# peleiden/librubiks

Hardware: AMD Instinct MI355X
Metric: cube node-expansions/sec (12-child fan-out) at 1M-state batch (higher is better)
Workload: dtype u8

## Files before the change

librubiks_amd/csrc/rk_mcts.hip:

```cpp
#include <hip/hip_runtime.h>
#include <algorithm>
#include <climits>
#include <cmath>
#include <cstdlib>
#include <cstring>
#include <vector>

#include "../../include/rubiks_hip.h"
#include "rk_device.h"
#include "rk_error.h"
#include "rk_kernels.h"

namespace rk {

struct MctsDev {
	int T;
	uint32_t cap1;
	uint32_t tmask;
	uint32_t max_path;
	double c, nu;
	uint32_t *states;
	uint8_t *nodes;
	uint32_t *table;
	int32_t *path_nodes; uint8_t *path_actions;
	int32_t *tree;
	uint32_t *children; int32_t *child_idx; uint8_t *child_new;
};

enum { TR_PLEN = 0, TR_NSTATES, TR_MAXSTATES, TR_SIMS, TR_SOLVE_ACTION, TR_SOLVE_LEAF, TR_READY, TR_FLAGS , TR_INTS = 8 };
enum { MCTS_ERR_PATH = 1, MCTS_ERR_LINK = 2, MCTS_ERR_NOT_EXPANDED = 3 };
__host__ __device__ inline int flags_done(int f) { return f & 0xFF; }
__host__ __device__ inline int flags_solved(int f) { return (f >> 8) & 0xFF; }
__host__ __device__ inline int flags_error(int f) { return (f >> 16) & 0xFF; }

struct TreeRec { int32_t v[TR_INTS]; };

__device__ __forceinline__ TreeRec load_tree(const int32_t *tree, int t)
{
	const u32x4 a = reinterpret_cast<const u32x4 *>(tree)[2 * t], b = reinterpret_cast<const u32x4 *>(tree)[2 * t + 1];
	return TreeRec{{(int32_t)a.x, (int32_t)a.y, (int32_t)a.z, (int32_t)a.w, (int32_t)b.x, (int32_t)b.y, (int32_t)b.z, (int32_t)b.w}};
}

constexpr int NODE_BYTES = 512;
constexpr int OFF_EXPANDED = 0, OFF_V = 8, OFF_N = 16, OFF_NB = 64, OFF_P = 112, OFF_W = 208, OFF_L = 304, OFF_STAMP = 400, OFF_SUMN = 448, OFF_SQRTN = 456;

struct Node {
	uint8_t *p;
	__device__ __forceinline__ uint32_t &expanded() const { return *reinterpret_cast<uint32_t *>(p + OFF_EXPANDED); }
	__device__ __forceinline__ double &V() const { return *reinterpret_cast<double *>(p + OFF_V); }
	__device__ __forceinline__ int32_t *N() const { return reinterpret_cast<int32_t *>(p + OFF_N); }
	__device__ __forceinline__ int32_t *nb() const { return reinterpret_cast<int32_t *>(p + OFF_NB); }
	__device__ __forceinline__ double *P() const { return reinterpret_cast<double *>(p + OFF_P); }
	__device__ __forceinline__ double *W() const { return reinterpret_cast<double *>(p + OFF_W); }
	__device__ __forceinline__ double *L() const { return reinterpret_cast<double *>(p + OFF_L); }
	__device__ __forceinline__ int32_t *stamp() const { return reinterpret_cast<int32_t *>(p + OFF_STAMP); }
	__device__ __forceinline__ int32_t *sumN() const { return reinterpret_cast<int32_t *>(p + OFF_SUMN); }
	__device__ __forceinline__ double &sqrtN() const { return *reinterpret_cast<double *>(p + OFF_SQRTN); }
};

__device__ __forceinline__ Node node_of(const MctsDev &d, size_t node0, int idx)
{
	return Node{d.nodes + (node0 + (size_t)idx) * NODE_BYTES};
}

__device__ __forceinline__ uint32_t mcts_hash(const uint32_t s[5])
{
	uint64_t h = 0x9E3779B97F4A7C15ull;
	#pragma unroll
	for (int j = 0; j < 5; j++) {
		h ^= s[j];
		h *= 0xFF51AFD7ED558CCDull;
		h ^= h >> 29;
	}
	return (uint32_t)(h ^ (h >> 32));
}

__device__ __forceinline__ bool same5(const uint32_t a[5], const uint32_t *p)
{
	return ((a[0] ^ p[0]) | (a[1] ^ p[1]) | (a[2] ^ p[2]) | (a[3] ^ p[3]) | (a[4] ^ p[4])) == 0;
}

template <int N> __device__ __forceinline__ int dpp_ror_i(int v)
{
	return __builtin_amdgcn_update_dpp(v, v, 0x120 + N, 0xF, 0xF, false);
}
template <int N> __device__ __forceinline__ double dpp_ror_d(double v)
{
	const long long b = __double_as_longlong(v);
	const int lo = dpp_ror_i<N>((int)(b & 0xFFFFFFFFll)), hi = dpp_ror_i<N>((int)(b >> 32));
	return __longlong_as_double(((long long)hi << 32) | (unsigned int)lo);
}
__device__ __forceinline__ int row_sum_i(int v)
{
	v += dpp_ror_i<8>(v); v += dpp_ror_i<4>(v); v += dpp_ror_i<2>(v); v += dpp_ror_i<1>(v);
	return v;
}
__device__ __forceinline__ float row_max_f(float v)
{
	#define RK_STEP(N) v = fmaxf(v, __int_as_float(dpp_ror_i<N>(__float_as_int(v))))
	RK_STEP(8); RK_STEP(4); RK_STEP(2); RK_STEP(1);
	#undef RK_STEP
	return v;
}
template <int N> __device__ __forceinline__ double dpp_ror_d_fresh(double v)
{
	const long long b = __double_as_longlong(v);
	const int lo = __builtin_amdgcn_mov_dpp((int)(b & 0xFFFFFFFFll), 0x120 + N, 0xF, 0xF, false);
	const int hi = __builtin_amdgcn_mov_dpp((int)(b >> 32), 0x120 + N, 0xF, 0xF, false);
	return __longlong_as_double(((long long)hi << 32) | (unsigned int)lo);
}
__device__ __forceinline__ double max_f64_raw(double a, double b)
{
	double r;
	asm("v_max_f64 %0, %1, %2" : "=v"(r) : "v"(a), "v"(b));
	return r;
}
__device__ __forceinline__ double row_max_d(double v)
{
	#define RK_STEP(N) v = max_f64_raw(v, dpp_ror_d_fresh<N>(v))
	RK_STEP(8); RK_STEP(4); RK_STEP(2); RK_STEP(1);
	#undef RK_STEP
	return v;
}
__device__ __forceinline__ void fence_wave_to_wave()
{
	__builtin_amdgcn_fence(__ATOMIC_RELEASE, "workgroup");
	__builtin_amdgcn_fence(__ATOMIC_ACQUIRE, "workgroup");
}

__global__ __launch_bounds__(64)
void k_mcts_root(MctsDev d, const uint32_t *starts, const int32_t *max_states)
{
	const int t = blockIdx.x, lane = threadIdx.x;
	uint32_t s[5];
	#pragma unroll
	for (int j = 0; j < 5; j++) s[j] = starts[(size_t)t * 5 + j];
	if (lane == 0) {
		uint32_t *st = d.states + ((size_t)t * d.cap1 + 1) * 5;
		#pragma unroll
		for (int j = 0; j < 5; j++) st[j] = s[j];
		d.table[(size_t)t * (d.tmask + 1) + (mcts_hash(s) & d.tmask)] = 1u;
		int32_t *tr = d.tree + (size_t)t * TR_INTS;
		tr[TR_NSTATES] = 1;
		tr[TR_MAXSTATES] = max_states[t];
		d.path_nodes[(size_t)t * d.max_path] = 1;
		tr[TR_PLEN] = 1;
		tr[TR_SIMS] = 0;
		tr[TR_READY] = 0;
		tr[TR_SOLVE_ACTION] = -1;
		tr[TR_SOLVE_LEAF] = -1;
		const bool solved = is_solved5(s);
		tr[TR_FLAGS] = solved ? (1 | (2 << 8)) : 0;
	}
}

__global__ void k_mcts_set_root_pv(MctsDev d, const float *probs, const float *values)
{
	const int i = blockIdx.x * blockDim.x + threadIdx.x;
	if (i >= d.T * 12) return;
	const int t = i / 12, k = i - 12 * t;
	const Node root = node_of(d, (size_t)t * d.cap1, 1);
	root.P()[k] = (double)probs[i];
	if (k == 0) root.V() = (double)values[t];
}

__global__ void k_mcts_gather_roots(MctsDev d, uint32_t *out)
{
	const int i = blockIdx.x * blockDim.x + threadIdx.x;
	if (i >= d.T * 5) return;
	const int t = i / 5, j = i - 5 * t;
	out[i] = d.states[((size_t)t * d.cap1 + 1) * 5 + j];
}

__device__ __forceinline__ void expand_leaf_body(const MctsDev &d, const u32x4 *s_act, int t, int lane, int n, int max_states, int flags, int leaf)
{
	const bool active = lane < 12;
	const size_t cbase = (size_t)t * 12 + lane;
	int32_t *trw = d.tree + (size_t)t * TR_INTS;
	if (n + 12 > max_states) {
		if (active) d.child_new[cbase] = 0;
		if (lane == 0) { trw[TR_FLAGS] = flags | 1; trw[TR_READY] = 1; }
		return;
	}
	const size_t node0 = (size_t)t * d.cap1;
	uint32_t s[5];
	#pragma unroll
	for (int j = 0; j < 5; j++) s[j] = d.states[(node0 + leaf) * 5 + j];
	uint32_t tab[12];
	load_action_table(s_act, active ? (uint32_t)lane : 0u, tab);
	move5(s, tab);

	uint32_t *table = d.table + (size_t)t * (d.tmask + 1);
	uint32_t slot = mcts_hash(s) & d.tmask;
	int idx = 0;
	if (active) {
		for (;;) {
			const uint32_t e = table[slot];
			if (e == 0u) break;
			if (same5(s, d.states + (node0 + e) * 5)) { idx = (int)e; break; }
			slot = (slot + 1) & d.tmask;
		}
	}
	const bool is_new = active && idx == 0;
	const unsigned long long newmask = __ballot(is_new);
	if (is_new) {
		idx = n + 1 + __popcll(newmask & ((1ull << lane) - 1ull));
		while (atomicCAS(&table[slot], 0u, (uint32_t)idx) != 0u) slot = (slot + 1) & d.tmask;
		#pragma unroll
		for (int j = 0; j < 5; j++) d.states[(node0 + idx) * 5 + j] = s[j];
	}
	if (active) {
		#pragma unroll
		for (int j = 0; j < 5; j++) d.children[cbase * 5 + j] = s[j];
		d.child_idx[cbase] = idx;
		d.child_new[cbase] = is_new ? 1 : 0;
		node_of(d, node0, leaf).nb()[lane] = idx;
		node_of(d, node0, idx).nb()[lane ^ 1] = leaf;
	}
	const unsigned long long solvedmask = __ballot(active && is_solved5(s));
	if (solvedmask != 0ull && lane == __ffsll((long long)solvedmask) - 1) {
		trw[TR_FLAGS] = (flags & 0xFF) | (1 << 8);
		trw[TR_SOLVE_ACTION] = lane;
		trw[TR_SOLVE_LEAF] = idx;
	}
	if (lane == 0) {
		node_of(d, node0, leaf).expanded() = 1u;
		trw[TR_NSTATES] = n + __popcll(newmask);
		trw[TR_READY] = 1;
	}
}

__global__ __launch_bounds__(64)
void k_mcts_expand(MctsDev d)
{
	__shared__ u32x4 s_act[36];
	const int t = blockIdx.x, lane = threadIdx.x;
	stage_action_tables(s_act, lane);
	__syncthreads();
	const TreeRec tr = load_tree(d.tree, t);
	if (tr.v[TR_FLAGS] & 0xFF) {
		if (lane < 12) d.child_new[(size_t)t * 12 + lane] = 0;
		return;
	}
	if (tr.v[TR_READY]) return;
	const int leaf = d.path_nodes[(size_t)t * d.max_path + tr.v[TR_PLEN] - 1];
	expand_leaf_body(d, s_act, t, lane, tr.v[TR_NSTATES], tr.v[TR_MAXSTATES], tr.v[TR_FLAGS], leaf);
}

template <int IN>
__device__ __forceinline__ float net_scalar(const void *p, size_t i)
{
	if (IN == 2) return __builtin_bit_cast(float, (uint32_t)reinterpret_cast<const uint16_t *>(p)[i] << 16);
	return reinterpret_cast<const float *>(p)[i];
}

template <int IN>
__device__ __forceinline__ void child_policy(const void *probs, size_t row, int stride, float out[12])
{
	#pragma unroll
	for (int k = 0; k < 12; k++) out[k] = net_scalar<IN>(probs, row * (size_t)stride + k);
	if (IN == 0) return;
	float m = out[0];
	#pragma unroll
	for (int k = 1; k < 12; k++) m = out[k] > m ? out[k] : m;
	#pragma unroll
	for (int k = 0; k < 12; k++) out[k] = expf(out[k] - m);
	const float a0 = (out[0] + out[8]) + out[4], a1 = (out[1] + out[9]) + out[5];
	const float a2 = (out[2] + out[10]) + out[6], a3 = (out[3] + out[11]) + out[7];
	const float sum = (a0 + a2) + (a1 + a3);
	#pragma unroll
	for (int k = 0; k < 12; k++) out[k] = out[k] / sum;
}

template <int IN>
__global__ __launch_bounds__(64)
void k_mcts_backup_select(MctsDev d, const void *probs, const void *values, int p_stride, int v_stride, int ahead_limit, int first_tree)
{
	__shared__ u32x4 s_act[36];
	const int t = blockIdx.x + first_tree, lane = threadIdx.x;
	if (ahead_limit != 0) stage_action_tables(s_act, lane);
	const bool active = lane < 12;
	const size_t node0 = (size_t)t * d.cap1;
	const size_t cbase = (size_t)t * 12 + lane;
	const int32_t *pnodes = d.path_nodes + (size_t)t * d.max_path;
	uint8_t *pacts = d.path_actions + (size_t)t * d.max_path;
	const TreeRec tr = load_tree(d.tree, t);
	int32_t *trw = d.tree + (size_t)t * TR_INTS;
	const int is_done = flags_done(tr.v[TR_FLAGS]), tree_solved = flags_solved(tr.v[TR_FLAGS]);
	const int plen = tr.v[TR_PLEN], sims_before = tr.v[TR_SIMS];
	const int idx = active ? d.child_idx[cbase] : 0;
	const bool is_new = active && d.child_new[cbase] != 0;
	const size_t rbase = (size_t)blockIdx.x * 12 + lane;
	const float vf = active ? net_scalar<IN>(values, rbase * (size_t)v_stride) : 0.0f;
	if (is_done) {
		if (ahead_limit != 0 && active) d.child_new[cbase] = 0;
		return;
	}
	if (!tr.v[TR_READY]) {
		if (lane == 0) trw[TR_FLAGS] = tr.v[TR_FLAGS] | 1 | (MCTS_ERR_NOT_EXPANDED << 16);
		return;
	}
	if (lane == 0) trw[TR_READY] = 0;
	const int leaf = pnodes[plen - 1];
	const double v = (double)vf;
	if (is_new) {
		const Node child = node_of(d, node0, idx);
		child.V() = v;
		float pk[12];
		child_policy<IN>(probs, rbase, p_stride, pk);
		#pragma unroll
		for (int k = 0; k < 12; k++) {
			child.P()[k] = (double)pk[k];
			child.W()[k] = v;
		}
	}
	float bestf = is_new ? vf : -INFINITY;
	bestf = __int_as_float(__builtin_amdgcn_readfirstlane(__float_as_int(row_max_f(bestf))));
	const bool has_new = __ballot(is_new) != 0ull;
	const double best = (double)bestf;
	if (active) node_of(d, node0, leaf).W()[lane] = is_new ? v : node_of(d, node0, idx).V();

	const int sim = sims_before + 1;
	for (int e = lane; e < plen - 1; e += 64) {
		const int act = pacts[e];
		const Node nd = node_of(d, node0, pnodes[e]);
		const double w = nd.W()[act];
		const int cnt = nd.N()[act];
		const int last = atomicExch(&nd.stamp()[act], sim);
		if (has_new && best > w) nd.W()[act] = best;
		if (last != sim) {
			nd.N()[act] = cnt + 1;
			const int total = atomicAdd(nd.sumN(), 1) + 1;
			atomicMax(reinterpret_cast<unsigned long long *>(&nd.sqrtN()), (unsigned long long)__double_as_longlong(sqrt((double)total)));
		}
		nd.L()[act] = 0.0;
		node_of(d, node0, pnodes[e + 1]).L()[act ^ 1] = 0.0;
	}
	if (lane == 0) trw[TR_SIMS] = sim;
	if (tree_solved) {
		if (lane == 0) {
			pacts[plen - 1] = (uint8_t)tr.v[TR_SOLVE_ACTION];
			trw[TR_FLAGS] = tr.v[TR_FLAGS] | 1;
		}
		if (ahead_limit != 0 && active) d.child_new[cbase] = 0;
		return;
	}
	fence_wave_to_wave();

	int cur = 1, len = 1, owed_lane = -1;
	for (;;) {
		const Node nd = node_of(d, node0, cur);
		const int col = lane < 12 ? lane : 11;
		const uint32_t expanded = nd.expanded();
		const double sqrtN = nd.sqrtN();
		const int nA = nd.N()[col];
		const double pA = nd.P()[col], wA = nd.W()[col];
		double lval = nd.L()[col];
		const int nb = nd.nb()[col];
		if (lane == owed_lane) { lval += d.nu; nd.L()[col] = lval; }
		if (!expanded) break;
		double x = -INFINITY;
		int best_a;
		{
			double U = d.c * pA;
			U = U * sqrtN;
			U = U / (double)(1 + nA);
			const double Q = wA - lval;
			x = active ? U + Q : -INFINITY;
		}
		const double mx = row_max_d(x);
		best_a = __ffsll((long long)(__ballot(x == mx) & 0xFFFull)) - 1;
		const int next = __builtin_amdgcn_readlane(nb, best_a);
		if (lane == best_a) nd.L()[col] = lval + d.nu;
		owed_lane = best_a ^ 1;
		if (lane == 0) {
			pacts[len - 1] = (uint8_t)best_a;
			d.path_nodes[(size_t)t * d.max_path + len] = next;
		}
		len++;
		cur = next;
		if (len >= (int)d.max_path || next <= 0) {
			if (lane == 0) trw[TR_FLAGS] = tr.v[TR_FLAGS] | 1 | ((next <= 0 ? MCTS_ERR_LINK : MCTS_ERR_PATH) << 16);
			break;
		}
	}
	if (lane == 0) trw[TR_PLEN] = len;
	const bool broke_on_error = len >= (int)d.max_path || cur <= 0;
	if (ahead_limit != 0 && !broke_on_error && (ahead_limit < 0 || sim < ahead_limit)) {
		fence_wave_to_wave();
		expand_leaf_body(d, s_act, t, lane, tr.v[TR_NSTATES], tr.v[TR_MAXSTATES], tr.v[TR_FLAGS], cur);
	} else if (ahead_limit != 0 && active) {
		d.child_new[cbase] = 0;
	}
}


__global__ __launch_bounds__(256)
void k_mcts_rehash(MctsDev d)
{
	const int t = blockIdx.y;
	const int n = d.tree[(size_t)t * TR_INTS + TR_NSTATES];
	const size_t node0 = (size_t)t * d.cap1;
	uint32_t *table = d.table + (size_t)t * (d.tmask + 1);
	for (int idx = 1 + blockIdx.x * blockDim.x + threadIdx.x; idx <= n; idx += gridDim.x * blockDim.x) {
		uint32_t s[5];
		#pragma unroll
		for (int j = 0; j < 5; j++) s[j] = d.states[(node0 + idx) * 5 + j];
		uint32_t slot = mcts_hash(s) & d.tmask;
		while (atomicCAS(&table[slot], 0u, (uint32_t)idx) != 0u) slot = (slot + 1) & d.tmask;
	}
}

__global__ void k_mcts_set_budgets(MctsDev d, const int32_t *max_states)
{
	const int t = blockIdx.x * blockDim.x + threadIdx.x;
	if (t >= d.T) return;
	int32_t *tr = d.tree + (size_t)t * TR_INTS;
	tr[TR_MAXSTATES] = max_states[t];
	const int f = tr[TR_FLAGS];
	if (flags_done(f) && !flags_solved(f) && !flags_error(f) && tr[TR_NSTATES] + 12 <= max_states[t]) {
		tr[TR_FLAGS] = f & ~0xFF;
		tr[TR_READY] = 0;
	}
}

__global__ __launch_bounds__(256)
void k_mcts_complete(MctsDev d)
{
	__shared__ u32x4 s_act[36];
	stage_action_tables(s_act, threadIdx.x);
	__syncthreads();
	const int t = blockIdx.y;
	const int32_t *tr = d.tree + (size_t)t * TR_INTS;
	if (flags_solved(tr[TR_FLAGS]) != 1) return;
	const int n = tr[TR_NSTATES];
	const size_t node0 = (size_t)t * d.cap1;
	const uint32_t *table = d.table + (size_t)t * (d.tmask + 1);
	const int a = threadIdx.x & 15;
	for (int idx = 1 + (blockIdx.x * blockDim.x + threadIdx.x) / 16; idx <= n; idx += gridDim.x * blockDim.x / 16) {
		const Node leaf = node_of(d, node0, idx);
		if (a >= 12 || leaf.expanded()) continue;
		uint32_t s[5];
		#pragma unroll
		for (int j = 0; j < 5; j++) s[j] = d.states[(node0 + idx) * 5 + j];
		uint32_t tab[12];
		load_action_table(s_act, (uint32_t)a, tab);
		move5(s, tab);
		uint32_t slot = mcts_hash(s) & d.tmask;
		int child = 0;
		for (;;) {
			const uint32_t e = table[slot];
			if (e == 0u) break;
			if (same5(s, d.states + (node0 + e) * 5)) { child = (int)e; break; }
			slot = (slot + 1) & d.tmask;
		}
		leaf.nb()[a] = child;
		if (child) node_of(d, node0, child).nb()[a ^ 1] = idx;
	}
}

struct BfsDev {
	uint32_t *claim;
	int32_t *from;
	uint8_t *act;
	int32_t *front[2];
	int32_t *len;
	uint8_t *actions;
};

__device__ __forceinline__ int ld_i32(const int32_t *p) { return __hip_atomic_load(p, __ATOMIC_RELAXED, __HIP_MEMORY_SCOPE_AGENT); }
__device__ __forceinline__ uint32_t ld_u32(const uint32_t *p) { return __hip_atomic_load(p, __ATOMIC_RELAXED, __HIP_MEMORY_SCOPE_AGENT); }

__global__ __launch_bounds__(1024)
void k_mcts_bfs(MctsDev d, BfsDev b)
{
	__shared__ int s_wave[16];
	__shared__ int s_count, s_found;
	const int t = blockIdx.x, tid = threadIdx.x, lane = tid & 63, wv = tid >> 6;
	const int32_t *tr = d.tree + (size_t)t * TR_INTS;
	const int goal = tr[TR_SOLVE_LEAF];
	if (flags_solved(tr[TR_FLAGS]) != 1 || goal <= 1) {
		if (tid == 0) b.len[t] = -1;
		return;
	}
	const size_t node0 = (size_t)t * d.cap1;
	uint32_t *claim = b.claim + node0;
	int32_t *from = b.from + node0;
	uint8_t *act = b.act + node0;
	int32_t *cur = b.front[0] + node0, *nxt = b.front[1] + node0;
	if (tid == 0) { cur[0] = 1; from[1] = -1; s_found = 0; }
	__syncthreads();
	int fsize = 1, depth = 0;
	while (fsize > 0) {
		const long long total = 12ll * fsize;
		for (long long e = tid; e < total; e += 1024) {
			const int v = ld_i32(cur + e / 12), a = (int)(e % 12);
			const int w = node_of(d, node0, v).nb()[a];
			if (w > 0 && ld_i32(from + w) == 0) atomicMin(claim + w, (uint32_t)e);
		}
		__syncthreads();
		if (tid == 0) s_count = 0;
		__syncthreads();
		for (long long base = 0; base < total; base += 1024) {
			const long long e = base + tid;
			int v = 0, a = 0, w = 0;
			bool win = false;
			if (e < total) {
				v = ld_i32(cur + e / 12); a = (int)(e % 12);
				w = node_of(d, node0, v).nb()[a];
				win = w > 0 && ld_i32(from + w) == 0 && ld_u32(claim + w) == (uint32_t)e;
			}
			const unsigned long long m = __ballot(win);
			if (lane == 0) s_wave[wv] = __popcll(m);
			__syncthreads();
			int before = 0, tot = 0;
			#pragma unroll
			for (int k = 0; k < 16; k++) { const int c = s_wave[k]; before += k < wv ? c : 0; tot += c; }
			const int at = s_count + before + __popcll(m & ((1ull << lane) - 1ull));
			if (win) {
				nxt[at] = w;
				__hip_atomic_store(from + w, v, __ATOMIC_RELAXED, __HIP_MEMORY_SCOPE_AGENT);
				act[w] = (uint8_t)a;
				if (w == goal) s_found = 1;
			}
			__syncthreads();
			if (tid == 0) s_count += tot;
			__syncthreads();
		}
		depth++;
		fsize = s_count;
		int32_t *sw = cur; cur = nxt; nxt = sw;
		if (s_found) break;
		__syncthreads();
	}
	if (tid == 0) {
		if (!s_found || depth > (int)d.max_path) { b.len[t] = -1; return; }
		uint8_t *out = b.actions + (size_t)t * d.max_path;
		int v = goal;
		for (int k = depth - 1; k >= 0; k--) {
			out[k] = __hip_atomic_load(act + v, __ATOMIC_RELAXED, __HIP_MEMORY_SCOPE_AGENT);
			v = ld_i32(from + v);
		}
		b.len[t] = depth;
	}
}

}

using namespace rk;

struct rk_mcts {
	MctsDev d{};
	size_t capacity = 0;
	std::vector<void *> allocs;
	uint32_t *starts_dev = nullptr;
	int32_t *max_states_dev = nullptr;
	bool ready = false;
	int ahead_limit = 0;
	bool ahead = false;
	int32_t *tree_host = nullptr;
	BfsDev bfs{};
	std::vector<void *> bfs_allocs;
	bool bfs_valid = false;
};

namespace {

template <typename T>
int mcts_alloc(rk_mcts *h, T **p, size_t count)
{
	void *q = nullptr;
	RK_HIP(hipMalloc(&q, count * sizeof(T) + 16));
	h->allocs.push_back(q);
	*p = static_cast<T *>(q);
	return RK_OK;
}

inline unsigned nblocks(size_t n, unsigned per = 256) { return (unsigned)((n + per - 1) / per); }

inline bool capturing(hipStream_t st)
{
	if (st == nullptr) return false;
	hipStreamCaptureStatus cap = hipStreamCaptureStatusNone;
	if (hipStreamIsCapturing(st, &cap) != hipSuccess) { (void)hipGetLastError(); return false; }
	return cap != hipStreamCaptureStatusNone;
}

hipError_t strided_copy(void *dst, size_t dpitch, const void *src, size_t spitch, size_t width, size_t rows, hipStream_t st)
{
	if (rows > 4096) return hipMemcpy2DAsync(dst, dpitch, src, spitch, width, rows, hipMemcpyDeviceToDevice, st);
	for (size_t r = 0; r < rows; r++) {
		const hipError_t e = hipMemcpyAsync((char *)dst + r * dpitch, (const char *)src + r * spitch, width, hipMemcpyDeviceToDevice, st);
		if (e != hipSuccess) return e;
	}
	return hipSuccess;
}

}

extern "C" {

int rk_mcts_create(rk_mcts_t **out, int n_trees, size_t capacity_per_tree, size_t max_path)
{
	if (!out) return fail(RK_EINVAL, "rk_mcts_create: null out pointer");
	if (n_trees < 1 || n_trees > (1 << 20)) return fail(RK_EINVAL, "rk_mcts_create: n_trees %d out of range", n_trees);
	if (capacity_per_tree < 13 || capacity_per_tree > 0x3FFFFFF0ull) return fail(RK_EINVAL, "rk_mcts_create: capacity %zu out of range", capacity_per_tree);
	if (max_path < 2 || max_path > (1u << 30)) return fail(RK_EINVAL, "rk_mcts_create: max_path %zu out of range", max_path);
	rk_mcts *h = new rk_mcts();
	h->capacity = capacity_per_tree;
	MctsDev &d = h->d;
	d.T = n_trees;
	d.cap1 = (uint32_t)(capacity_per_tree + 1);
	uint64_t ts = 64;
	while (ts < 2ull * d.cap1) ts <<= 1;
	d.tmask = (uint32_t)(ts - 1);
	d.max_path = (uint32_t)max_path;
	const size_t T = (size_t)n_trees, rows = T * d.cap1;
	int e = RK_OK;
	#define A(ptr, cnt) if (!e) e = mcts_alloc(h, &d.ptr, (cnt))
	A(states, rows * 5); A(nodes, (rows + 1) * NODE_BYTES);
	A(table, T * (size_t)ts);
	A(path_nodes, T * max_path); A(path_actions, T * max_path);
	A(tree, T * TR_INTS + 16);
	A(children, T * 12 * 5 + 64); A(child_idx, T * 12); A(child_new, T * 12);
	#undef A
	if (!e) e = mcts_alloc(h, &h->starts_dev, T * 5);
	if (!e) e = mcts_alloc(h, &h->max_states_dev, T);
	if (!e && hipHostMalloc((void **)&h->tree_host, T * TR_INTS * sizeof(int32_t), hipHostMallocDefault) != hipSuccess) { (void)hipGetLastError(); h->tree_host = nullptr; }
	if (e) { rk_mcts_destroy(h); return e; }
	*out = h;
	return RK_OK;
}

int rk_mcts_destroy(rk_mcts_t *h)
{
	if (!h) return RK_OK;
	for (void *p : h->allocs) (void)hipFree(p);
	for (void *p : h->bfs_allocs) (void)hipFree(p);
	if (h->tree_host != nullptr) (void)hipHostFree(h->tree_host);
	delete h;
	return RK_OK;
}

int rk_mcts_reset(rk_mcts_t *h, const int8_t *h_start_states, const long long *h_max_states, double c, double nu, void *stream)
{
	if (!h || !h_start_states) return fail(RK_EINVAL, "rk_mcts_reset: null argument");
	hipStream_t st = (hipStream_t)stream;
	MctsDev &d = h->d;
	const size_t T = (size_t)d.T, rows = T * d.cap1;
	d.c = c;
	d.nu = nu;
	std::vector<int32_t> ms(T);
	for (size_t t = 0; t < T; t++) {
		long long m = h_max_states ? h_max_states[t] : (long long)h->capacity;
		if (m > (long long)h->capacity) m = (long long)h->capacity;
		ms[t] = (int32_t)(m < 0 ? 0 : m);
	}
	RK_HIP(hipMemsetAsync(d.nodes, 0, rows * NODE_BYTES, st));
	RK_HIP(hipMemsetAsync(d.table, 0, T * ((size_t)d.tmask + 1) * sizeof(uint32_t), st));
	RK_HIP(hipMemsetAsync(d.child_new, 0, T * 12, st));
	RK_HIP(hipMemsetAsync(d.child_idx, 0, T * 12 * sizeof(int32_t), st));
	RK_HIP(hipMemsetAsync(d.children, 0, (T * 12 * 5) * sizeof(uint32_t), st));
	RK_HIP(hipMemcpyAsync(h->max_states_dev, ms.data(), T * sizeof(int32_t), hipMemcpyHostToDevice, st));
	RK_HIP(hipMemcpyAsync(h->starts_dev, h_start_states, T * STATE_BYTES, hipMemcpyHostToDevice, st));
	hipLaunchKernelGGL(k_mcts_root, dim3(d.T), dim3(64), 0, st, d, h->starts_dev, h->max_states_dev);
	RK_HIP(hipGetLastError());
	RK_HIP(hipStreamSynchronize(st));
	h->ready = true;
	h->ahead = false;
	return RK_OK;
}


int rk_mcts_grow(rk_mcts_t *h, size_t new_capacity, size_t new_max_path, const long long *h_max_states, void *stream)
{
	if (!h || !h->ready) return fail(RK_ESTATE, "rk_mcts_grow: reset the engine first");
	if (new_capacity < h->capacity || new_capacity > 0x3FFFFFF0ull) return fail(RK_EINVAL, "rk_mcts_grow: capacity %zu out of range (now %zu)", new_capacity, h->capacity);
	if (new_max_path < h->d.max_path) new_max_path = h->d.max_path;
	if (new_max_path > (1u << 30)) return fail(RK_EINVAL, "rk_mcts_grow: max_path %zu out of range", new_max_path);
	hipStream_t st = (hipStream_t)stream;
	const MctsDev old = h->d;
	MctsDev d = old;
	const size_t T = (size_t)d.T;
	d.cap1 = (uint32_t)(new_capacity + 1);
	uint64_t ts = 64;
	while (ts < 2ull * d.cap1) ts <<= 1;
	d.tmask = (uint32_t)(ts - 1);
	d.max_path = (uint32_t)new_max_path;
	const size_t rows = T * d.cap1;
	std::vector<void *> fresh;
	auto get = [&](size_t bytes) -> void * { void *q = nullptr; if (hipMalloc(&q, bytes + 16) != hipSuccess) return nullptr; fresh.push_back(q); return q; };
	const bool pool = d.cap1 != old.cap1, paths = d.max_path != old.max_path;
	if (pool) {
		d.states = (uint32_t *)get(rows * 5 * sizeof(uint32_t));
		d.nodes = (uint8_t *)get((rows + 1) * NODE_BYTES);
		d.table = (uint32_t *)get(T * (size_t)ts * sizeof(uint32_t));
	}
	if (paths) {
		d.path_nodes = (int32_t *)get(T * new_max_path * sizeof(int32_t));
		d.path_actions = (uint8_t *)get(T * new_max_path);
	}
	if ((pool && (!d.states || !d.nodes || !d.table)) || (paths && (!d.path_nodes || !d.path_actions))) {
		for (void *q : fresh) (void)hipFree(q);
		(void)hipGetLastError();
		return fail(RK_ECAPACITY, "rk_mcts_grow: no device memory for %d trees of %zu states", d.T, new_capacity);
	}
	std::vector<int32_t> ms(T);
	for (size_t t = 0; t < T; t++) {
		long long m = h_max_states ? h_max_states[t] : (long long)new_capacity;
		if (m > (long long)new_capacity) m = (long long)new_capacity;
		ms[t] = (int32_t)(m < 0 ? 0 : m);
	}
	auto fill = [&]() -> hipError_t {
		#define RK_TRY(call) do { const hipError_t e_ = (call); if (e_ != hipSuccess) return e_; } while (0)
		if (pool) {
			RK_TRY(hipMemsetAsync(d.nodes, 0, rows * NODE_BYTES, st));
			RK_TRY(hipMemsetAsync(d.table, 0, T * (size_t)ts * sizeof(uint32_t), st));
			RK_TRY(strided_copy(d.states, (size_t)d.cap1 * STATE_BYTES, old.states, (size_t)old.cap1 * STATE_BYTES, (size_t)old.cap1 * STATE_BYTES, T, st));
			RK_TRY(strided_copy(d.nodes, (size_t)d.cap1 * NODE_BYTES, old.nodes, (size_t)old.cap1 * NODE_BYTES, (size_t)old.cap1 * NODE_BYTES, T, st));
		}
		if (paths) {
			RK_TRY(strided_copy(d.path_nodes, new_max_path * 4, old.path_nodes, (size_t)old.max_path * 4, (size_t)old.max_path * 4, T, st));
			RK_TRY(strided_copy(d.path_actions, new_max_path, old.path_actions, (size_t)old.max_path, (size_t)old.max_path, T, st));
		}
		if (pool) {
			hipLaunchKernelGGL(k_mcts_rehash, dim3(std::min<unsigned>(nblocks(old.cap1), 4096u), d.T), dim3(256), 0, st, d);
			RK_TRY(hipGetLastError());
		}
		RK_TRY(hipMemcpyAsync(h->max_states_dev, ms.data(), T * sizeof(int32_t), hipMemcpyHostToDevice, st));
		hipLaunchKernelGGL(k_mcts_set_budgets, dim3(nblocks(T)), dim3(256), 0, st, d, h->max_states_dev);
		RK_TRY(hipGetLastError());
		RK_TRY(hipStreamSynchronize(st));
		#undef RK_TRY
		return hipSuccess;
	};
	if (const hipError_t e = fill(); e != hipSuccess) {
		(void)hipStreamSynchronize(st);
		for (void *q : fresh) (void)hipFree(q);
		(void)hipGetLastError();
		return fail(RK_EHIP, "rk_mcts_grow: %s", hipGetErrorString(e));
	}
	auto drop = [&](void *q) {
		for (size_t i = 0; i < h->allocs.size(); i++) if (h->allocs[i] == q) { h->allocs.erase(h->allocs.begin() + (long)i); break; }
		(void)hipFree(q);
	};
	if (pool) { drop(old.states); drop(old.nodes); drop(old.table); }
	if (paths) { drop(old.path_nodes); drop(old.path_actions); }
	for (void *q : fresh) h->allocs.push_back(q);
	h->d = d;
	h->capacity = new_capacity;
	h->ahead = false;
	for (void *q : h->bfs_allocs) (void)hipFree(q);
	h->bfs_allocs.clear();
	h->bfs = BfsDev{};
	h->bfs_valid = false;
	return RK_OK;
}

int rk_mcts_search_graph(rk_mcts_t *h, void *stream)
{
	if (!h || !h->ready) return fail(RK_ESTATE, "rk_mcts_search_graph: reset the engine first");
	hipStream_t st = (hipStream_t)stream;
	const MctsDev &d = h->d;
	const size_t T = (size_t)d.T, rows = T * d.cap1;
	if (h->bfs.claim == nullptr) {
		BfsDev b{};
		auto get = [&](size_t bytes) -> void * { void *q = nullptr; if (hipMalloc(&q, bytes + 16) != hipSuccess) return nullptr; h->bfs_allocs.push_back(q); return q; };
		b.claim = (uint32_t *)get(rows * 4); b.from = (int32_t *)get(rows * 4); b.act = (uint8_t *)get(rows);
		b.front[0] = (int32_t *)get(rows * 4); b.front[1] = (int32_t *)get(rows * 4);
		b.len = (int32_t *)get(T * 4); b.actions = (uint8_t *)get(T * (size_t)d.max_path);
		if (!b.claim || !b.from || !b.act || !b.front[0] || !b.front[1] || !b.len || !b.actions) {
			for (void *q : h->bfs_allocs) (void)hipFree(q);
			h->bfs_allocs.clear();
			(void)hipGetLastError();
			return fail(RK_ECAPACITY, "rk_mcts_search_graph: no device memory for the search scratch of %d trees", d.T);
		}
		h->bfs = b;
	}
	RK_HIP(hipMemsetAsync(h->bfs.claim, 0xFF, rows * 4, st));
	RK_HIP(hipMemsetAsync(h->bfs.from, 0, rows * 4, st));
	hipLaunchKernelGGL(k_mcts_complete, dim3(std::min<unsigned>(nblocks((size_t)d.cap1 * 16), 8192u), d.T), dim3(256), 0, st, d);
	hipLaunchKernelGGL(k_mcts_bfs, dim3(d.T), dim3(1024), 0, st, d, h->bfs);
	RK_HIP(hipGetLastError());
	h->bfs_valid = true;
	return RK_OK;
}

long long rk_mcts_graph_path(rk_mcts_t *h, int tree, long long *h_actions, size_t max_len, void *stream)
{
	if (!h || !h->ready) return fail(RK_ESTATE, "rk_mcts_graph_path: reset the engine first");
	if (!h->bfs_valid) return fail(RK_ESTATE, "rk_mcts_graph_path: call rk_mcts_search_graph first");
	const MctsDev &d = h->d;
	if (tree < 0 || tree >= d.T) return fail(RK_EINVAL, "rk_mcts_graph_path: tree %d out of range", tree);
	hipStream_t st = (hipStream_t)stream;
	int32_t len = -1;
	RK_HIP(hipMemcpyAsync(&len, h->bfs.len + tree, sizeof len, hipMemcpyDeviceToHost, st));
	RK_HIP(hipStreamSynchronize(st));
	if (len <= 0) return len < 0 ? -1 : 0;
	std::vector<uint8_t> acts((size_t)len);
	RK_HIP(hipMemcpyAsync(acts.data(), h->bfs.actions + (size_t)tree * d.max_path, (size_t)len, hipMemcpyDeviceToHost, st));
	RK_HIP(hipStreamSynchronize(st));
	for (size_t i = 0; i < (size_t)len && i < max_len; i++) if (h_actions) h_actions[i] = acts[i];
	return len;
}

int rk_mcts_set_expand_ahead(rk_mcts_t *h, long long sim_limit)
{
	if (!h) return fail(RK_EINVAL, "rk_mcts_set_expand_ahead: null handle");
	h->ahead_limit = sim_limit < 0 ? -1 : (sim_limit > INT_MAX ? INT_MAX : (int)sim_limit);
	return RK_OK;
}

int rk_mcts_roots_oh(rk_mcts_t *h, void *d_out, int out_dtype, void *stream)
{
	if (!h || !h->ready) return fail(RK_ESTATE, "rk_mcts_roots_oh: reset the engine first");
	MctsDev &d = h->d;
	if (out_dtype == RK_OH_STATES) {
		if (!d_out) return fail(RK_EINVAL, "rk_mcts_roots_oh: null output");
		hipLaunchKernelGGL(k_mcts_gather_roots, dim3(nblocks((size_t)d.T * 5)), dim3(256), 0, (hipStream_t)stream, d, (uint32_t *)d_out);
		RK_HIP(hipGetLastError());
		return RK_OK;
	}
	hipLaunchKernelGGL(k_mcts_gather_roots, dim3(nblocks((size_t)d.T * 5)), dim3(256), 0, (hipStream_t)stream, d, d.children);
	RK_HIP(hipGetLastError());
	return rk_as_oh(RK_REPR_2024, (const int8_t *)d.children, d_out, out_dtype, (size_t)d.T, stream);
}

int rk_mcts_set_root_pv(rk_mcts_t *h, const float *d_probs, const float *d_values, void *stream)
{
	if (!h || !h->ready) return fail(RK_ESTATE, "rk_mcts_set_root_pv: reset the engine first");
	if (!d_probs || !d_values) return fail(RK_EINVAL, "rk_mcts_set_root_pv: null pointer");
	hipLaunchKernelGGL(k_mcts_set_root_pv, dim3(nblocks((size_t)h->d.T * 12)), dim3(256), 0, (hipStream_t)stream, h->d, d_probs, d_values);
	RK_HIP(hipGetLastError());
	return RK_OK;
}

int rk_mcts_expand(rk_mcts_t *h, void *stream)
{
	if (!h || !h->ready) return fail(RK_ESTATE, "rk_mcts_expand: reset the engine first");
	if (!capturing((hipStream_t)stream)) {
		const bool skip = h->ahead;
		h->ahead = false;
		if (skip) return RK_OK;
	}
	hipLaunchKernelGGL(k_mcts_expand, dim3(h->d.T), dim3(64), 0, (hipStream_t)stream, h->d);
	RK_HIP(hipGetLastError());
	return RK_OK;
}

int rk_mcts_children_oh(rk_mcts_t *h, void *d_out, int out_dtype, void *stream)
{
	if (!h || !h->ready) return fail(RK_ESTATE, "rk_mcts_children_oh: reset the engine first");
	if (out_dtype == RK_OH_STATES) {
		if (!d_out) return fail(RK_EINVAL, "rk_mcts_children_oh: null output");
		RK_HIP(hipMemcpyAsync(d_out, h->d.children, (size_t)h->d.T * 12 * STATE_BYTES, hipMemcpyDeviceToDevice, (hipStream_t)stream));
		return RK_OK;
	}
	return rk_as_oh(RK_REPR_2024, (const int8_t *)h->d.children, d_out, out_dtype, (size_t)h->d.T * 12, stream);
}

int rk_mcts_backup_select(rk_mcts_t *h, const float *d_probs, const float *d_values, void *stream)
{
	if (!h || !h->ready) return fail(RK_ESTATE, "rk_mcts_backup_select: reset the engine first");
	if (!d_probs || !d_values) return fail(RK_EINVAL, "rk_mcts_backup_select: null pointer");
	hipLaunchKernelGGL(k_mcts_backup_select<0>, dim3(h->d.T), dim3(64), 0, (hipStream_t)stream, h->d, (const void *)d_probs, (const void *)d_values, 12, 1, h->ahead_limit, 0);
	RK_HIP(hipGetLastError());
	if (!capturing((hipStream_t)stream)) h->ahead = h->ahead_limit != 0;
	return RK_OK;
}

static int backup_select_logits_impl(rk_mcts_t *h, int first_tree, int n_trees, const void *d_logits, int logits_stride, const void *d_values, int values_stride,
                                     int dtype, void *stream)
{
	if (!h || !h->ready) return fail(RK_ESTATE, "rk_mcts_backup_select_logits: reset the engine first");
	if (!d_logits || !d_values) return fail(RK_EINVAL, "rk_mcts_backup_select_logits: null pointer");
	if (logits_stride < 12 || values_stride < 1) return fail(RK_EINVAL, "rk_mcts_backup_select_logits: strides are in elements, at least 12 and 1");
	if (first_tree < 0 || n_trees < 1 || first_tree + n_trees > h->d.T)
		return fail(RK_EINVAL, "rk_mcts_backup_select_logits_range: trees %d..%d outside 0..%d", first_tree, first_tree + n_trees, h->d.T);
	if (dtype == RK_OH_F32)
		hipLaunchKernelGGL(k_mcts_backup_select<1>, dim3(n_trees), dim3(64), 0, (hipStream_t)stream, h->d, d_logits, d_values, logits_stride, values_stride, h->ahead_limit, first_tree);
	else if (dtype == RK_OH_BF16)
		hipLaunchKernelGGL(k_mcts_backup_select<2>, dim3(n_trees), dim3(64), 0, (hipStream_t)stream, h->d, d_logits, d_values, logits_stride, values_stride, h->ahead_limit, first_tree);
	else
		return fail(RK_EINVAL, "rk_mcts_backup_select_logits: logits and values must be float32 or bfloat16");
	RK_HIP(hipGetLastError());
	if (!capturing((hipStream_t)stream)) h->ahead = h->ahead_limit != 0;
	return RK_OK;
}

int rk_mcts_backup_select_logits(rk_mcts_t *h, const void *d_logits, int logits_stride, const void *d_values, int values_stride, int dtype, void *stream)
{
	return backup_select_logits_impl(h, 0, h ? h->d.T : 1, d_logits, logits_stride, d_values, values_stride, dtype, stream);
}

int rk_mcts_backup_select_logits_range(rk_mcts_t *h, int first_tree, int n_trees, const void *d_logits, int logits_stride, const void *d_values,
                                       int values_stride, int dtype, void *stream)
{
	return backup_select_logits_impl(h, first_tree, n_trees, d_logits, logits_stride, d_values, values_stride, dtype, stream);
}

const int8_t *rk_mcts_children(rk_mcts_t *h)
{
	return h ? reinterpret_cast<const int8_t *>(h->d.children) : nullptr;
}

int rk_mcts_status(rk_mcts_t *h, long long *h_status, void *stream)
{
	if (!h || !h->ready || !h_status) return fail(RK_EINVAL, "rk_mcts_status: bad argument");
	hipStream_t st = (hipStream_t)stream;
	const MctsDev &d = h->d;
	const size_t T = (size_t)d.T;
	std::vector<int32_t> pageable;
	int32_t *rec = h->tree_host;
	if (rec == nullptr) { pageable.resize(T * TR_INTS); rec = pageable.data(); }
	RK_HIP(hipMemcpyAsync(rec, d.tree, T * TR_INTS * sizeof(int32_t), hipMemcpyDeviceToHost, st));
	RK_HIP(hipStreamSynchronize(st));
	for (size_t t = 0; t < T; t++) {
		const int32_t *tr = rec + t * TR_INTS;
		long long *r = h_status + 6 * t;
		r[0] = flags_done(tr[TR_FLAGS]); r[1] = flags_solved(tr[TR_FLAGS]); r[2] = tr[TR_NSTATES]; r[3] = tr[TR_SIMS]; r[4] = tr[TR_PLEN];
		r[5] = flags_error(tr[TR_FLAGS]);
	}
	return RK_OK;
}

int rk_mcts_export(rk_mcts_t *h, int tree, size_t first, size_t count, int8_t *h_states, long long *h_neighbors,
                   uint8_t *h_leaves, double *h_P, double *h_V, long long *h_N, double *h_W, double *h_L, void *stream)
{
	if (!h || !h->ready) return fail(RK_ESTATE, "rk_mcts_export: reset the engine first");
	const MctsDev &d = h->d;
	if (tree < 0 || tree >= d.T) return fail(RK_EINVAL, "rk_mcts_export: tree %d out of range", tree);
	if (first + count > d.cap1) return fail(RK_EINVAL, "rk_mcts_export: rows outside the pool");
	if (count == 0) return RK_OK;
	hipStream_t st = (hipStream_t)stream;
	const size_t r0 = (size_t)tree * d.cap1 + first;
	if (h_states) RK_HIP(hipMemcpyAsync(h_states, d.states + r0 * 5, count * STATE_BYTES, hipMemcpyDeviceToHost, st));
	std::vector<uint8_t> rec;
	const bool want_nodes = h_neighbors || h_leaves || h_P || h_V || h_N || h_W || h_L;
	if (want_nodes) {
		rec.resize(count * NODE_BYTES);
		RK_HIP(hipMemcpyAsync(rec.data(), d.nodes + r0 * NODE_BYTES, count * NODE_BYTES, hipMemcpyDeviceToHost, st));
	}
	RK_HIP(hipStreamSynchronize(st));
	for (size_t i = 0; want_nodes && i < count; i++) {
		const uint8_t *p = rec.data() + i * NODE_BYTES;
		uint32_t expanded;
		memcpy(&expanded, p + OFF_EXPANDED, 4);
		if (h_leaves) h_leaves[i] = expanded ? 0 : 1;
		if (h_V) memcpy(h_V + i, p + OFF_V, 8);
		if (h_P) memcpy(h_P + i * 12, p + OFF_P, 96);
		if (h_W) memcpy(h_W + i * 12, p + OFF_W, 96);
		if (h_L) memcpy(h_L + i * 12, p + OFF_L, 96);
		for (int k = 0; k < 12; k++) {
			int32_t v;
			if (h_neighbors) { memcpy(&v, p + OFF_NB + 4 * k, 4); h_neighbors[i * 12 + k] = v; }
			if (h_N) { memcpy(&v, p + OFF_N + 4 * k, 4); h_N[i * 12 + k] = v; }
		}
	}
	return RK_OK;
}

long long rk_mcts_path(rk_mcts_t *h, int tree, long long *h_actions, long long *h_nodes, size_t max_len, void *stream)
{
	if (!h || !h->ready) return fail(RK_ESTATE, "rk_mcts_path: reset the engine first");
	const MctsDev &d = h->d;
	if (tree < 0 || tree >= d.T) return fail(RK_EINVAL, "rk_mcts_path: tree %d out of range", tree);
	hipStream_t st = (hipStream_t)stream;
	int32_t tr[TR_INTS];
	RK_HIP(hipMemcpyAsync(tr, d.tree + (size_t)tree * TR_INTS, sizeof tr, hipMemcpyDeviceToHost, st));
	RK_HIP(hipStreamSynchronize(st));
	const int32_t plen = tr[TR_PLEN];
	const int solved = flags_solved(tr[TR_FLAGS]);
	if (plen < 1) return fail(RK_ESTATE, "rk_mcts_path: empty path");
	std::vector<int32_t> nodes((size_t)plen);
	std::vector<uint8_t> acts((size_t)plen);
	RK_HIP(hipMemcpyAsync(nodes.data(), d.path_nodes + (size_t)tree * d.max_path, (size_t)plen * 4, hipMemcpyDeviceToHost, st));
	RK_HIP(hipMemcpyAsync(acts.data(), d.path_actions + (size_t)tree * d.max_path, (size_t)plen, hipMemcpyDeviceToHost, st));
	RK_HIP(hipStreamSynchronize(st));
	const size_t n_act = solved == 1 ? (size_t)plen : (solved == 2 ? 0 : (size_t)plen - 1);
	for (size_t i = 0; i < n_act && i < max_len; i++) if (h_actions) h_actions[i] = acts[i];
	for (size_t i = 0; i < (size_t)plen && i < max_len; i++) if (h_nodes) h_nodes[i] = nodes[i];
	return (long long)n_act;
}

}
```

Measured before the change: 24.93 billion.

## Speculatively re-descend MCTS tree along previous path in parallel windows

Adds a speculative descent to the backup/select kernel. It evaluates the UCT choice for up to 64 nodes of the previous path at once (four nodes per wave, 16 lanes each) and accepts the longest prefix whose best action matches the old path. It then resumes the serial descent from the first divergence. This aims to replace a serial chain of dependent node loads with batched parallel loads. The cost is extra register pressure, repeat-node detection, and more complex virtual-loss bookkeeping. An environment variable can switch back to the serial descent.

```diff
diff --git a/librubiks_amd/csrc/rk_mcts.hip b/librubiks_amd/csrc/rk_mcts.hip
--- a/librubiks_amd/csrc/rk_mcts.hip
+++ b/librubiks_amd/csrc/rk_mcts.hip
@@ -42,6 +42,7 @@
 }
 
 constexpr int NODE_BYTES = 512;
+constexpr int SPEC_W = 64;
 constexpr int OFF_EXPANDED = 0, OFF_V = 8, OFF_N = 16, OFF_NB = 64, OFF_P = 112, OFF_W = 208, OFF_L = 304, OFF_STAMP = 400, OFF_SUMN = 448, OFF_SQRTN = 456;
 
 struct Node {
@@ -274,7 +275,7 @@
 
 template <int IN>
 __global__ __launch_bounds__(64)
-void k_mcts_backup_select(MctsDev d, const void *probs, const void *values, int p_stride, int v_stride, int ahead_limit, int first_tree)
+void k_mcts_backup_select(MctsDev d, const void *probs, const void *values, int p_stride, int v_stride, int ahead_limit, int first_tree, int speculative)
 {
 	__shared__ u32x4 s_act[36];
 	const int t = blockIdx.x + first_tree, lane = threadIdx.x;
@@ -321,9 +322,12 @@
 	if (active) node_of(d, node0, leaf).W()[lane] = is_new ? v : node_of(d, node0, idx).V();
 
 	const int sim = sims_before + 1;
+	int win_node = lane == plen - 1 ? leaf : 0, win_act = 0xFF;
 	for (int e = lane; e < plen - 1; e += 64) {
 		const int act = pacts[e];
-		const Node nd = node_of(d, node0, pnodes[e]);
+		const int pnode = pnodes[e];
+		if (e < SPEC_W) { win_node = pnode; win_act = act; }
+		const Node nd = node_of(d, node0, pnode);
 		const double w = nd.W()[act];
 		const int cnt = nd.N()[act];
 		const int last = atomicExch(&nd.stamp()[act], sim);
@@ -348,7 +352,112 @@
 	fence_wave_to_wave();
 
 	int cur = 1, len = 1, owed_lane = -1;
-	for (;;) {
+	bool open = true;
+	if (speculative) {
+		const int row = lane >> 4, col16 = lane & 15, colc = col16 < 12 ? col16 : 11;
+		int w0 = 0, carry_act = -1;
+		for (;;) {
+			const int cnt0 = min(SPEC_W, plen - w0);
+			if (w0 > 0) {
+				win_node = lane < cnt0 ? pnodes[w0 + lane] : 0;
+				win_act = w0 + lane < plen - 1 && lane < cnt0 ? (int)pacts[w0 + lane] : 0xFF;
+			}
+			int win_prev = __shfl_up(win_act, 1);
+			if (lane == 0) win_prev = carry_act;
+			int s_node[SPEC_W / 4], s_n[SPEC_W / 4], s_nb[SPEC_W / 4], s_best[SPEC_W / 4];
+			uint32_t s_exp[SPEC_W / 4];
+			double s_sqrt[SPEC_W / 4], s_p[SPEC_W / 4], s_w[SPEC_W / 4], s_l[SPEC_W / 4];
+			#pragma unroll
+			for (int k = 0; k < SPEC_W / 4; k++) {
+				s_node[k] = 0; s_n[k] = 0; s_nb[k] = 0; s_best[k] = 0; s_exp[k] = 0u;
+				s_sqrt[k] = 0.0; s_p[k] = 0.0; s_w[k] = 0.0; s_l[k] = 0.0;
+				if (4 * k < cnt0) {
+					s_node[k] = __shfl(win_node, 4 * k + row);
+					const Node nd = node_of(d, node0, s_node[k]);
+					s_exp[k] = nd.expanded();
+					s_sqrt[k] = nd.sqrtN();
+					s_n[k] = nd.N()[colc];
+					s_p[k] = nd.P()[colc];
+					s_w[k] = nd.W()[colc];
+					s_l[k] = nd.L()[colc];
+					s_nb[k] = nd.nb()[colc];
+				}
+			}
+			bool repeat = false;
+			for (int j = 0; j < cnt0 - 1; j++)
+				repeat |= j < lane && __builtin_amdgcn_readlane(win_node, j) == win_node;
+			const unsigned long long rmask = __ballot(repeat && lane < cnt0);
+			const int cnt = rmask != 0ull ? min(cnt0, __ffsll((long long)rmask) - 1) : cnt0;
+			unsigned long long agree = 0ull;
+			#pragma unroll
+			for (int k = 0; k < SPEC_W / 4; k++) {
+				if (4 * k < cnt) {
+					const int a_old = __shfl(win_act, 4 * k + row), a_prev = __shfl(win_prev, 4 * k + row);
+					double lval = s_l[k];
+					if (col16 == (a_prev ^ 1)) lval += d.nu;
+					double U = d.c * s_p[k];
+					U = U * s_sqrt[k];
+					U = U / (double)(1 + s_n[k]);
+					const double Q = s_w[k] - lval;
+					const double x = col16 < 12 ? U + Q : -INFINITY;
+					const double mx = row_max_d(x);
+					const unsigned long long hold = __ballot(x == mx);
+					const int best_a = __ffs((int)((uint32_t)(hold >> (16 * row)) & 0xFFFu)) - 1;
+					s_l[k] = lval;
+					s_best[k] = best_a;
+					const unsigned long long ok = __ballot(s_exp[k] != 0u && best_a == a_old);
+					agree |= ((ok & 1ull) | ((ok >> 15) & 2ull) | ((ok >> 30) & 4ull) | ((ok >> 45) & 8ull)) << (4 * k);
+				}
+			}
+			const int run = ~agree != 0ull ? __ffsll((long long)~agree) - 1 : 64;
+			const int m = min(cnt, run);
+			const bool ended = m < cnt;
+			const int last = ended ? m : m - 1;
+			int f_exp = 0, f_best = 0, f_next = 0, f_node = 0;
+			#pragma unroll
+			for (int k = 0; k < SPEC_W / 4; k++) {
+				if (4 * k <= last) {
+					const int a_prev = __shfl(win_prev, 4 * k + row);
+					const bool chose = s_exp[k] != 0u && col16 == s_best[k];
+					if (4 * k + row <= last && (chose || col16 == (a_prev ^ 1)))
+						node_of(d, node0, s_node[k]).L()[colc] = chose ? s_l[k] + d.nu : s_l[k];
+					if (ended && k == m >> 2) {
+						const int l0 = 16 * (m & 3);
+						f_exp = (int)__builtin_amdgcn_readlane((int)s_exp[k], l0);
+						f_best = __builtin_amdgcn_readlane(s_best[k], l0);
+						f_node = __builtin_amdgcn_readlane(s_node[k], l0);
+						f_next = __builtin_amdgcn_readlane(s_nb[k], l0 + (f_best & 15));
+					}
+				}
+			}
+			fence_wave_to_wave();
+			if (!ended) {
+				carry_act = __builtin_amdgcn_readlane(win_act, m - 1);
+				w0 += m;
+				continue;
+			}
+			const int f = w0 + m;
+			if (!f_exp) {
+				cur = f_node;
+				len = f + 1;
+				open = false;
+				break;
+			}
+			if (lane == 0) {
+				pacts[f] = (uint8_t)f_best;
+				d.path_nodes[(size_t)t * d.max_path + f + 1] = f_next;
+			}
+			owed_lane = f_best ^ 1;
+			len = f + 2;
+			cur = f_next;
+			if (len >= (int)d.max_path || f_next <= 0) {
+				if (lane == 0) trw[TR_FLAGS] = tr.v[TR_FLAGS] | 1 | ((f_next <= 0 ? MCTS_ERR_LINK : MCTS_ERR_PATH) << 16);
+				open = false;
+			}
+			break;
+		}
+	}
+	while (open) {
 		const Node nd = node_of(d, node0, cur);
 		const int col = lane < 12 ? lane : 11;
 		const uint32_t expanded = nd.expanded();
@@ -558,6 +667,7 @@
 	bool ready = false;
 	int ahead_limit = 0;
 	bool ahead = false;
+	bool speculative = true;
 	int32_t *tree_host = nullptr;
 	BfsDev bfs{};
 	std::vector<void *> bfs_allocs;
@@ -608,6 +718,7 @@
 	if (max_path < 2 || max_path > (1u << 30)) return fail(RK_EINVAL, "rk_mcts_create: max_path %zu out of range", max_path);
 	rk_mcts *h = new rk_mcts();
 	h->capacity = capacity_per_tree;
+	if (const char *e = std::getenv("RK_MCTS_DESCENT")) h->speculative = std::strcmp(e, "serial") != 0;
 	MctsDev &d = h->d;
 	d.T = n_trees;
 	d.cap1 = (uint32_t)(capacity_per_tree + 1);
@@ -863,7 +974,7 @@
 {
 	if (!h || !h->ready) return fail(RK_ESTATE, "rk_mcts_backup_select: reset the engine first");
 	if (!d_probs || !d_values) return fail(RK_EINVAL, "rk_mcts_backup_select: null pointer");
-	hipLaunchKernelGGL(k_mcts_backup_select<0>, dim3(h->d.T), dim3(64), 0, (hipStream_t)stream, h->d, (const void *)d_probs, (const void *)d_values, 12, 1, h->ahead_limit, 0);
+	hipLaunchKernelGGL(k_mcts_backup_select<0>, dim3(h->d.T), dim3(64), 0, (hipStream_t)stream, h->d, (const void *)d_probs, (const void *)d_values, 12, 1, h->ahead_limit, 0, (int)h->speculative);
 	RK_HIP(hipGetLastError());
 	if (!capturing((hipStream_t)stream)) h->ahead = h->ahead_limit != 0;
 	return RK_OK;
@@ -878,9 +989,9 @@
 	if (first_tree < 0 || n_trees < 1 || first_tree + n_trees > h->d.T)
 		return fail(RK_EINVAL, "rk_mcts_backup_select_logits_range: trees %d..%d outside 0..%d", first_tree, first_tree + n_trees, h->d.T);
 	if (dtype == RK_OH_F32)
-		hipLaunchKernelGGL(k_mcts_backup_select<1>, dim3(n_trees), dim3(64), 0, (hipStream_t)stream, h->d, d_logits, d_values, logits_stride, values_stride, h->ahead_limit, first_tree);
+		hipLaunchKernelGGL(k_mcts_backup_select<1>, dim3(n_trees), dim3(64), 0, (hipStream_t)stream, h->d, d_logits, d_values, logits_stride, values_stride, h->ahead_limit, first_tree, (int)h->speculative);
 	else if (dtype == RK_OH_BF16)
-		hipLaunchKernelGGL(k_mcts_backup_select<2>, dim3(n_trees), dim3(64), 0, (hipStream_t)stream, h->d, d_logits, d_values, logits_stride, values_stride, h->ahead_limit, first_tree);
+		hipLaunchKernelGGL(k_mcts_backup_select<2>, dim3(n_trees), dim3(64), 0, (hipStream_t)stream, h->d, d_logits, d_values, logits_stride, values_stride, h->ahead_limit, first_tree, (int)h->speculative);
 	else
 		return fail(RK_EINVAL, "rk_mcts_backup_select_logits: logits and values must be float32 or bfloat16");
 	RK_HIP(hipGetLastError());
```

After: 24.93 billion, median of 2. About the same (+0.0%).
